# SAR-Research-Lab/lvt

Measured on AMD Instinct MI355X. Metric: stereo frames/sec (KITTI-shaped 1241x376), per-frame SE3 vs CPU ref, higher is better.
Workload: dtype u8/f64

## Files before the change

### lvt_amd/csrc/k_features.hip

```cpp
#include "lvt_dev.h"
#include "lvt_handover.h"
#include "lvt_math.h"
#include <type_traits>

namespace lvt {

__constant__ signed char c_brief[256][4] = {
#include "../../include/lvt_brief256_pattern.inc"
};
constexpr signed char BRIEF_TABLE[256][4] = {
#include "../../include/lvt_brief256_pattern.inc"
};
constexpr int brief_max_offset() {
    int m = 0;
    for (int i = 0; i < 256; i++)
        for (int k = 0; k < 4; k++) m = (BRIEF_TABLE[i][k] > m) ? BRIEF_TABLE[i][k] : (-BRIEF_TABLE[i][k] > m) ? -BRIEF_TABLE[i][k] : m;
    return m;
}

constexpr int TS_W = 64, TS_H = 16, HALO = 4;
constexpr int TILE_W = TS_W + 2 * HALO;
constexpr int TILE_H = TS_H + 2 * HALO;

typedef short s16x2 __attribute__((ext_vector_type(2)));
// ... 1786 lines not shown
constexpr int BR_WIN_DW = BR_ROWS * BR_DW, BR_LOADS = (BR_WIN_DW + 63) / 64;
template <bool BV>
__global__ __launch_bounds__(256) void k_brief(SeqArg<BV> sa, int par, seq_t publish_seq) {
    int plane, bx;
    const int planes = brief_plane_of_block(plane, bx);
    const Seq &S = sa.at(plane / gridDim.y);
    const int eye = plane % gridDim.y;
    const FrameBuf &FB = S.fb[par];
    const Feat &F = FB.feat[eye];
    const bool poison = FB.fc->poison != 0;
    const int n = poison ? 0 : *F.n;
    const int lane = lane_id();
    const int wpb = blockDim.x >> 6;
    __shared__ uint32_t s_win[4][BR_WIN_DW + 64];
    uint32_t *win = s_win[wave_id()];
    typedef uint16_t __attribute__((may_alias)) u16_alias;
    const u16_alias *win16 = reinterpret_cast<const u16_alias *>(win);
    const int W = S.prm.W, H = S.prm.H, ppd = S.plane_pitch >> 1;
    const uint32_t *box32 = reinterpret_cast<const uint32_t *>(FB.boxsum[eye]);
    int goff[BR_LOADS];
#pragma unroll
    for (int i = 0; i < BR_LOADS; i++) {
        const int e = min(lane + 64 * i, BR_WIN_DW - 1);
        goff[i] = (e / BR_DW) * ppd + (e % BR_DW);
    }
    int ta[4], tb[4];
    signed char tq[4][4];
#pragma unroll
    for (int w = 0; w < 4; w++) {
        const signed char *t = c_brief[64 * w + 8 * (lane >> 3) + 7 - (lane & 7)];
        tq[w][0] = t[0], tq[w][1] = t[1], tq[w][2] = t[2], tq[w][3] = t[3];
        ta[w] = (t[0] + BR_R) * (2 * BR_DW) + t[1] + BR_R;
        tb[w] = (t[2] + BR_R) * (2 * BR_DW) + t[3] + BR_R;
    }
    auto inside = [&](int cy, int cx) { return cx - BR_R >= 0 && cx + BR_R < W && cy - BR_R >= 0 && cy + BR_R < H; };
    int i, i_end;
    const int stride = brief_key_points_of_wave(planes, bx, wpb, n, i, i_end);
    uint32_t v[BR_LOADS];
    int cy = 0, cx = 0;
    bool fast = false;
    auto fetch = [&](int cy_, int cx_) {
        typedef const uint32_t __attribute__((address_space(1))) gu32;
        gu32 *src = (gu32 *)(box32 + (size_t)(cy_ - BR_R) * ppd + ((cx_ - BR_R) >> 1));
#pragma unroll
        for (int k = 0; k < BR_LOADS; k++) v[k] = src[goff[k]];
    };
    if (i < i_end) {
        brief_centre(F, i, cy, cx);
        fast = inside(cy, cx);
        if (fast) fetch(cy, cx);
    }
    for (; i < i_end; i += stride) {
        uint64_t word[4];
        const int inext = i + stride;
        int ncy = 0, ncx = 0;
        bool nfast = false;
        if (inext < i_end) {
            brief_centre(F, inext, ncy, ncx);
            nfast = inside(ncy, ncx);
        }
        if (fast) {
#pragma unroll
            for (int k = 0; k < BR_LOADS; k++) win[lane + 64 * k] = v[k];
            if (nfast) fetch(ncy, ncx);
            const int odd = (cx - BR_R) & 1;
#pragma unroll
            for (int w = 0; w < 4; w++) {
                const int a = win16[ta[w] + odd], b = win16[tb[w] + odd];
                word[w] = __ballot(a < b);
            }
        } else {
            if (nfast) fetch(ncy, ncx);
#pragma unroll
            for (int w = 0; w < 4; w++) {
                const int a = box_at(S, FB, eye, cy + tq[w][0], cx + tq[w][1]);
                const int b = box_at(S, FB, eye, cy + tq[w][2], cx + tq[w][3]);
                word[w] = __ballot(a < b);
            }
        }
        if (lane < 4) F.desc[(size_t)i * 4 + lane] = (lane == 0) ? word[0] : (lane == 1) ? word[1] : (lane == 2) ? word[2] : word[3];
        cy = ncy, cx = ncx, fast = nfast;
    }
    if (publish_seq) last_block_publishes(S, FB, publish_seq);
}


constexpr int BI_R = BR_R + 4, BI_ROWS = 2 * BI_R + 1;
constexpr int BI_DW = 16;
constexpr int BI_G = 13;
constexpr int BI_PATCH_DW = BI_ROWS * BI_DW, BI_LOADS = (BI_PATCH_DW + 63) / 64;
constexpr int BI_GROUPS = BI_ROWS * BI_G, BI_GLOOPS = (BI_GROUPS + 63) / 64;
template <bool BV>
__global__ __launch_bounds__(256) void k_brief_img(SeqArg<BV> sa, int par, seq_t publish_seq) {
    int plane, bx;
    const int planes = brief_plane_of_block(plane, bx);
    const Seq &S = sa.at(plane / gridDim.y);
    const int eye = plane % gridDim.y;
    const FrameBuf &FB = S.fb[par];
    const Feat &F = FB.feat[eye];
    const bool poison = FB.fc->poison != 0;
    const int n = poison ? 0 : *F.n;
    const int lane = lane_id();
    const int wpb = blockDim.x >> 6;
    __shared__ uint32_t s_patch[4][BI_PATCH_DW + 64];
    __shared__ __attribute__((aligned(8))) uint2 s_hs[4][BI_GROUPS + 64];
    uint32_t *pat = s_patch[wave_id()];
    uint2 *hs = s_hs[wave_id()];
    typedef uint16_t __attribute__((may_alias)) u16_alias;
    const u16_alias *hs16 = reinterpret_cast<const u16_alias *>(hs);
    const int W = S.prm.W, H = S.prm.H;
    const uint8_t *img = wave_uniform(FB.fc->in.img[eye]);
    const int pitch = FB.fc->in.img_pitch;
    int goff[BI_LOADS];
#pragma unroll
    for (int i = 0; i < BI_LOADS; i++) {
        const int e = min(lane + 64 * i, BI_PATCH_DW - 1);
        goff[i] = (e / BI_DW) * (pitch >> 2) + (e % BI_DW);
    }
    int ta[4], tb[4];
    signed char tq[4][4];
#pragma unroll
    for (int w = 0; w < 4; w++) {
        const signed char *t = c_brief[64 * w + 8 * (lane >> 3) + 7 - (lane & 7)];
        tq[w][0] = t[0], tq[w][1] = t[1], tq[w][2] = t[2], tq[w][3] = t[3];
        ta[w] = (t[0] + BR_R) * (4 * BI_G) + t[1] + BR_R;
        tb[w] = (t[2] + BR_R) * (4 * BI_G) + t[3] + BR_R;
    }
    auto inside = [&](int cy, int cx) { return cx - BI_R >= 0 && ((cx - BI_R) & ~3) + 64 <= pitch && cx + BI_R < W && cy - BI_R >= 0 && cy + BI_R < H; };
    int i, i_end;
    const int stride = brief_key_points_of_wave(planes, bx, wpb, n, i, i_end);
    uint32_t v[BI_LOADS];
    int cy = 0, cx = 0;
    bool fast = false;
    auto fetch = [&](int cy_, int cx_) {
        typedef const uint32_t __attribute__((address_space(1))) gu32;
        gu32 *src = (gu32 *)(reinterpret_cast<const uint32_t *>(img + (size_t)(cy_ - BI_R) * pitch) + (((cx_ - BI_R) & ~3) >> 2));
#pragma unroll
        for (int k = 0; k < BI_LOADS; k++) v[k] = src[goff[k]];
    };
    auto box_slow = [&](int iy, int ix) -> int {
        int sum = 0;
        for (int y = max(iy - 4, 0); y <= min(iy + 4, H - 1); y++)
            for (int x = max(ix - 4, 0); x <= min(ix + 4, W - 1); x++) sum += img[(size_t)y * pitch + x];
        return sum;
    };
    if (i < i_end) {
        brief_centre(F, i, cy, cx);
        fast = inside(cy, cx);
        if (fast) fetch(cy, cx);
    }
    for (; i < i_end; i += stride) {
        uint64_t word[4];
        const int inext = i + stride;
        int ncy = 0, ncx = 0;
        bool nfast = false;
        if (inext < i_end) {
            brief_centre(F, inext, ncy, ncx);
            nfast = inside(ncy, ncx);
        }
        if (fast) {
#pragma unroll
            for (int k = 0; k < BI_LOADS; k++) pat[lane + 64 * k] = v[k];
            if (nfast) fetch(ncy, ncx);
#pragma unroll
            for (int k = 0; k < BI_GLOOPS; k++) {
                const int g = min(lane + 64 * k, BI_GROUPS - 1);
// ... 36 lines not shown
```

### lvt_amd/csrc/lvt_host.hip

```cpp
#define LVT_EXPORT_FUNCTIONS
#include "../../include/lvt_amd_ext.h"

#include "k_features.hip"
#include "k_track.hip"
#include "k_hamming.hip"
#include "k_lists.hip"
#include "k_rectify.hip"
#include "k_depthreg.hip"
#include "k_equalise.hip"
#include "k_state.hip"
#include "k_poseinfo.hip"
#include "lvt_odometry.h"

#include <atomic>
#include <cmath>
#include <chrono>
#include <cstdio>
#include <cstdlib>
#include <cstring>
#include <string>
#include <functional>
#include <vector>

namespace lvt {
// ... 45 lines not shown
    const size_t head = min((size_t)(((16 - ((uintptr_t)src & 15)) & 15) / sizeof(T)), n);
    const size_t nv = (n - head) / PER, tail0 = head + nv * PER;
    const size_t t0 = (size_t)blockIdx.x * blockDim.x + threadIdx.x, stride = (size_t)gridDim.x * blockDim.x;
    for (size_t v = t0; v < nv; v += stride) {
        Vec u;
        u.q = *reinterpret_cast<const uint4 *>(src + head + v * PER);
        T *d = dst + head + v * PER;
#pragma unroll
        for (size_t k = 0; k < PER; k++) d[k] = u.e[k];
    }
    if (t0 < head) dst[t0] = src[t0];
    if (t0 < n - tail0) dst[tail0 + t0] = src[tail0 + t0];
}
static void launch_stage_copy(hipStream_t st, const uint8_t *src, float *d_dst, size_t n, int fmt) {
    if (fmt == DEPTH_U16) hipLaunchKernelGGL(k_stage_copy<uint16_t>, dim3(256), dim3(256), 0, st, reinterpret_cast<const uint16_t *>(src), reinterpret_cast<uint16_t *>(d_dst), n);
    else hipLaunchKernelGGL(k_stage_copy<float>, dim3(256), dim3(256), 0, st, reinterpret_cast<const float *>(src), d_dst, n);
}

constexpr int MAX_DEVICES = 64;
static std::atomic<int> g_live_contexts[MAX_DEVICES];
static thread_local std::string g_snap_err;

constexpr uint64_t CTX_MAGIC = 0x4C56545F43545831ull, SLOT_MAGIC = 0x4C56545F534C5431ull;

struct Rectifier {
    int w = 0, h = 0, pitch = 0;
    int device = 0;
    float *d_map1 = nullptr, *d_map2 = nullptr;
    int2 *d_fix = nullptr;
    uint8_t *d_src = nullptr, *d_dst = nullptr;
};

struct HostStage {
    uint8_t *h = nullptr, *dev = nullptr;
    size_t second = 0;
};

struct Context {
    uint64_t magic = CTX_MAGIC;
    double host_enq_us = 0, host_wait_us = 0;
    long host_enq_n = 0, host_wait_n = 0;
    int gate_timeouts_seen = 0, gate_fatal_seen = 0;
    bool want_events = false, ordering_forced = false;
    hipEvent_t ev_switch = nullptr, ev_switch_e = nullptr;
    long test_gate_timeout = 0, switched_at = -1;
    long long planes_in_place = 0, planes_staged = 0;
    int device = 0;
    int B = 1;
    int launch_seqs = 0;
    int ring_seqs[8] = {};
    int sensor = 1;
    Params prm{};
    bool mixed = false;
    std::vector<Params> prms;
    std::vector<lvt_amd_params> in_prms;
    uint32_t *d_score_tab = nullptr, *d_cells_tab = nullptr;
    int n_score_wgs = 0, n_cells_wgs = 0;
    bool any_staged = false, any_strips = false;
    int max_cells = 0;
    const Params &seq_prm(int s) const { return mixed ? prms[s] : prm; }
    hipStream_t stream = nullptr;
    hipStream_t stream_f = nullptr;
    hipStream_t stream_e = nullptr;
    bool own_stream = false;
    std::vector<void *> allocs;
    const Seq *d_seqs = nullptr;
    std::vector<Seq> h_seqs;
    std::vector<Ctl *> d_ctl;
    Ctl *h_ctl = nullptr;
    Ctl *h_ctl_dev = nullptr;
    seq_t *h_done = nullptr, *h_done_dev = nullptr;
    PoseRec *h_pose = nullptr, *h_pose_dev = nullptr;
    seq_t *h_pose_done = nullptr, *h_pose_done_dev = nullptr;
    bool binned_lists = false;
    bool early_pose = true;
    bool early_pending = false;
    FrameArgs *h_fargs = nullptr;
    bool pose_info = false;
    lvt_amd_pose_info *h_pinfo = nullptr, *h_pinfo_dev = nullptr;
    hipEvent_t ev_done[RING] = {};
    bool events_only = false;
    CellOrder cell_order;
    bool feat_pack = true;
    int brief_from_image = 0;
    int score_pieces = 1;
    bool score_pieces_auto = true;
    double gate_balance_us = 0;
    int cells_raw_cap = RAW_CAP;
    unsigned cell_token = 0;
    int cell_split = 2;
    int lists_wgs_row = LISTS_WGS_ROW, lists_wgs_map = LISTS_WGS_MAP;
    int match_blocks_batch = 32;
    bool force_row_fallback = false;
    hipEvent_t ev_feat[NPAR] = {};
    hipEvent_t ev_depth = nullptr;
    bool depth_wait = false;
    std::function<void()> before_gather;
    uint8_t *d_img[NPAR][2] = {};
    HostStage stage[NPAR];
    float *d_depth[NPAR] = {};
    uint8_t *d_img_ring[RING][2] = {};
    float *d_depth_ring[RING] = {};
    HostStage stage_ring[RING];
    long long async_frames = 0;
    struct PendingFrame {
        bool valid = false, pulled = false;
        FrameArgs f{};
        const uint8_t *src[2] = {nullptr, nullptr};
        uint8_t *dst[2] = {nullptr, nullptr};
        int row_bytes = 0, pitch = 0;
    } pend;
    NextPull next_pull{};
    bool fuse_pull = true;
    long long fused_pulls = 0;
    int feature_cus = 0;
    float *d_ext[NPAR][2] = {};
    std::vector<Rectifier *> rect;
    std::vector<uint8_t *> d_rect;
    int n_rect = 0;
    bool has_rect(int s) const { return n_rect > 0 && rect[2 * (size_t)s] != nullptr; }
    std::vector<int> pixfmt;
    std::vector<uint8_t *> d_gray;
    int n_colour = 0;
    bool ring_converted[RING] = {};
    int fmt_of(int s) const { return n_colour > 0 ? pixfmt[(size_t)s] : PIX_GRAY8; }
    int bpp_of(int s) const { return pix_bpp(fmt_of(s)); }
    uint8_t *d_col[NPAR][2] = {};
    uint8_t *d_col_ring[RING][2] = {};
    int colour_pitch() const { return (prm.W * bpp_of(0) + 63) / 64 * 64; }
    std::vector<lvt_amd_depth_camera> depth_cam;
    std::vector<float *> d_reg;
    int n_depth_cam = 0;
    bool ring_registered[RING] = {};
    bool has_depth_cam(int s) const { return n_depth_cam > 0 && depth_cam[(size_t)s].width > 0; }
    std::vector<lvt_amd_equalisation> equal;
    std::vector<uint8_t *> d_eq;
    std::vector<uint8_t *> d_eq_lut;
    int n_equal = 0;
    bool ring_equalised[RING] = {};
    bool has_equal(int s) const { return n_equal > 0 && equal[(size_t)s].tiles_x > 0; }
    size_t depth_px() const { return has_depth_cam(0) ? (size_t)depth_cam[0].width * depth_cam[0].height : (size_t)prm.W * prm.H; }
    int depth_cols() const { return has_depth_cam(0) ? depth_cam[0].width : prm.W; }
    size_t depth_cap = 0, depth_ring_cap = 0;
    int pitch = 0;
    int *d_snap_status = nullptr;
    long enq = 0, done = 0;
    long delivered = 0;
    bool sync_call = false;
    int last_slot = 0, last_par = 0;
    std::string err;
    bool prof = false;
    static constexpr int PROF_SLOTS = 26;
    hipEvent_t ev[PROF_SLOTS][2] = {};
    bool ev_used[PROF_SLOTS] = {};
    double prof_ms[PROF_SLOTS] = {};
    long prof_calls[PROF_SLOTS] = {};

    void set_error(const std::string &s) { err = s; }
    long long ovf_done = -1, ovf_read_done = -1;
    bool capacity_report() const { return err.compare(0, 17, "capacity overflow") == 0; }

    template <typename T>
    T *dalloc_uncached(size_t n) {
        void *p = nullptr;
        size_t bytes = ((n * sizeof(T) + 255) / 256) * 256;
        if (bytes == 0) bytes = 256;
// ... 289 lines not shown
    c->device = device;
    DeviceGuard guard(c);
    try {
        c->count_in(device);
        c->B = B;
        c->sensor = sensor;
        c->prm = prm;
        c->mixed = mixed;
        if (mixed) c->prms = prms;
        c->in_prms.assign(in, in + prms.size());
        for (const Params &q : prms) {
            c->any_staged = c->any_staged || q.staged_th > 0;
            c->any_strips = c->any_strips || q.big_cell_strips != 0;
            c->max_cells = std::max(c->max_cells, q.n_cells);
        }
        HIPCHK(c, hipStreamCreateWithFlags(&c->stream, hipStreamNonBlocking));
        {
            int ncu = 0;
            if (B >= 2 && B <= 28) {
                int total = 0;
                if (hipDeviceGetAttribute(&total, hipDeviceAttributeMultiprocessorCount, device) == hipSuccess && total >= 64) ncu = total / 8 * 7;
            }
            if (const char *e = std::getenv("LVT_AMD_FEATURE_CUS")) ncu = (B >= 2) ? std::atoi(e) : 0;
            if (ncu > 0 && ncu < 1024) {
                uint32_t mask[32] = {};
                for (int i = 0; i < ncu; i++) mask[i >> 5] |= 1u << (i & 31);
                HIPCHK(c, hipExtStreamCreateWithCUMask(&c->stream_f, 32, mask));
                c->feature_cus = ncu;
            } else
                HIPCHK(c, hipStreamCreateWithFlags(&c->stream_f, hipStreamNonBlocking));
        }
        HIPCHK(c, hipStreamCreateWithFlags(&c->stream_e, hipStreamNonBlocking));
        c->own_stream = true;
        for (auto &e : c->ev_done) HIPCHK(c, hipEventCreateWithFlags(&e, hipEventDisableTiming));
        for (auto &e : c->ev_feat) HIPCHK(c, hipEventCreateWithFlags(&e, hipEventDisableTiming));
        HIPCHK(c, hipEventCreateWithFlags(&c->ev_depth, hipEventDisableTiming));
        HIPCHK(c, hipEventCreateWithFlags(&c->ev_switch, hipEventDisableTiming));
        HIPCHK(c, hipEventCreateWithFlags(&c->ev_switch_e, hipEventDisableTiming));
        if (const char *e = std::getenv("LVT_AMD_TEST_GATE_TIMEOUT")) c->test_gate_timeout = std::atol(e);
        {
            const char *o = std::getenv("LVT_AMD_ORDERING");
            if (o && std::strcmp(o, "events") == 0) c->events_only = true;
            else if (o && std::strcmp(o, "polling") == 0) c->events_only = false, c->ordering_forced = true;
            else c->events_only = B == 1 && c->live_on_device() > 1;
        }
        c->pitch = ((prm.W + 63) / 64) * 64;
        HIPCHK(c, hipHostMalloc((void **)&c->h_ctl, sizeof(Ctl) * B * RING, hipHostMallocCoherent));
        HIPCHK(c, hipHostGetDevicePointer((void **)&c->h_ctl_dev, c->h_ctl, 0));
        HIPCHK(c, hipHostMalloc((void **)&c->h_done, sizeof(seq_t) * B * RING, hipHostMallocCoherent));
        HIPCHK(c, hipHostGetDevicePointer((void **)&c->h_done_dev, c->h_done, 0));
        std::memset(c->h_done, 0, sizeof(seq_t) * B * RING);
        HIPCHK(c, hipHostMalloc((void **)&c->h_pose, sizeof(PoseRec) * B * RING, hipHostMallocCoherent));
        HIPCHK(c, hipHostGetDevicePointer((void **)&c->h_pose_dev, c->h_pose, 0));
        HIPCHK(c, hipHostMalloc((void **)&c->h_pose_done, sizeof(seq_t) * B * RING, hipHostMallocCoherent));
        HIPCHK(c, hipHostGetDevicePointer((void **)&c->h_pose_done_dev, c->h_pose_done, 0));
        std::memset(c->h_pose_done, 0, sizeof(seq_t) * B * RING);
        if (const char *e = std::getenv("LVT_AMD_SYNC_TAIL")) c->early_pose = std::strcmp(e, "wait") != 0;
        c->binned_lists = B > 1;
        if (const char *e = std::getenv("LVT_AMD_BINNED_LISTS")) c->binned_lists = std::atoi(e) != 0;
        if (const char *e = std::getenv("LVT_AMD_TEST_ROW_FALLBACK")) c->force_row_fallback = std::atoi(e) != 0;
        {
            int idx[CELLS_MAX], area[CELLS_MAX];
            for (int cc = 0; cc < prm.n_cells; cc++) {
                const int cx = cc % prm.cells_x, cy = cc / prm.cells_x;
                idx[cc] = cc;
                area[cc] = std::min(prm.cell_size, prm.W - cx * prm.cell_size) * std::min(prm.cell_size, prm.H - cy * prm.cell_size);
            }
            std::stable_sort(idx, idx + prm.n_cells, [&](int a, int b) { return area[a] > area[b]; });
            for (int cc = 0; cc < CELLS_MAX; cc++) c->cell_order.v[cc] = (uint8_t)(cc < prm.n_cells ? idx[cc] : 0);
        }
        if (std::getenv("LVT_AMD_NO_FEAT_PACK")) c->feat_pack = false;
        if (const char *e = std::getenv("LVT_AMD_BRIEF_FROM_IMAGE")) c->brief_from_image = std::atoi(e) ? 1 : 0;
        if (const char *e = std::getenv("LVT_AMD_SCORE_PIECES")) c->score_pieces = std::max(1, std::min(8, std::atoi(e))), c->score_pieces_auto = false;
        {
            int n_cu = 256;
            (void)hipDeviceGetAttribute(&n_cu, hipDeviceAttributeMultiprocessorCount, c->device);
            if (!mixed && !prm.big_cell_strips && prm.n_cells * 2 * B > n_cu) c->cells_raw_cap = RAW_CAP_SMALL;
            if (mixed && !c->any_strips && (int)cells_tab.size() > n_cu) c->cells_raw_cap = RAW_CAP_SMALL;
        }
        if (mixed) c->score_pieces = 1, c->score_pieces_auto = false;
        if (const char *e = std::getenv("LVT_AMD_CELL_SPLIT")) c->cell_split = std::max(0, std::min(SPLIT_MAX, std::atoi(e)));
        if (const char *e = std::getenv("LVT_AMD_CELLS_RAW_CAP")) c->cells_raw_cap = std::max(RAW_CAP_SMALL, std::min(RAW_CAP, std::atoi(e) & ~1));
        if (const char *e = std::getenv("LVT_AMD_FUSED_PULL")) c->fuse_pull = std::atoi(e) != 0;
        c->lists_wgs_row = c->lists_wgs_map = (B <= 16) ? 4 : 2;
        if (const char *e = std::getenv("LVT_AMD_LISTS_WGS")) {
            int r = 0, m = 0;
            const int got = std::sscanf(e, "%d,%d", &r, &m);
            if (got >= 1) c->lists_wgs_row = std::max(1, std::min(64, r));
            if (got >= 2) c->lists_wgs_map = std::max(1, std::min(64, m));
        }
        if (const char *e = std::getenv("LVT_AMD_MATCH_BLOCKS_BATCH")) c->match_blocks_batch = std::max(1, std::min(256, std::atoi(e)));
        HIPCHK(c, hipHostMalloc((void **)&c->h_fargs, sizeof(FrameArgs) * B * RING, hipHostMallocDefault));
        std::memset(c->h_fargs, 0, sizeof(FrameArgs) * B * RING);
        c->h_seqs.resize(B);
        c->d_ctl.resize(B);
        for (int s = 0; s < B; s++) {
            const Params &q = prms[mixed ? s : 0];
            const int pitch = ((q.W + 63) / 64) * 64;
            const size_t plane = (size_t)pitch * q.H;
            Seq &S = c->h_seqs[s];
            std::memset(&S, 0, sizeof(S));
            S.prm = q;
            S.ctl = c->d_ctl[s] = c->dalloc<Ctl>(1);
            S.plane_pitch = pitch;
            {
                size_t off = 0;
                for (int cc = 0; cc < q.n_cells; cc++) {
                    const int cx = cc % q.cells_x, cy = cc / q.cells_x;
                    const int cw = std::min(q.cell_size, q.W - cx * q.cell_size), ch = std::min(q.cell_size, q.H - cy * q.cell_size);
                    S.cell_scratch_off[cc] = off;
                    off += (size_t)cw * ch * 6;
                }
            }
            for (int e = 0; e < 2; e++) S.cell_scratch[e] = c->dalloc<uint32_t>((size_t)q.W * q.H * 6 + 64);
            for (int e = 0; e < 2; e++) {
                S.strip_kp[e] = q.big_cell_strips ? c->dalloc<uint32_t>((size_t)q.n_cells * STRIPS * RAW_CAP) : c->dalloc_uncached<uint32_t>((size_t)q.n_cells * SPLIT_MAX * SPLIT_KP_CAP);
                S.strip_n[e] = c->dalloc_uncached<int>((size_t)CELLS_MAX * STRIPS);
                S.cell_big[e] = c->dalloc<int>(CELLS_MAX);
            }
            S.lists_fb = c->dalloc<int>(2);
            for (int par = 0; par < NPAR; par++) {
                FrameBuf &FB = S.fb[par];
                FB.fc = c->dalloc<FeatCtl>(1);
                for (int e = 0; e < 2; e++) {
                    FB.score[e] = c->dalloc<uint8_t>(plane + 64);
                    FB.boxsum[e] = c->dalloc<uint16_t>(plane + 64);
                    {
                        const size_t tiles_x = (size_t)(q.W + TS_W - 1) / TS_W;
                        FB.seg_keys[e] = c->dalloc<uint32_t>((size_t)q.H * tiles_x * TS_W);
                        FB.seg_cnt[e] = c->dalloc<uint16_t>((size_t)q.H * tiles_x);
                    }
                    FB.cell_kp[e] = c->dalloc<float>((size_t)CELLS_MAX * CELL_OUT_CAP * 3);
                    FB.cell_n[e] = c->dalloc<int>(CELLS_MAX);
                    alloc_feat(c, FB.feat[e]);
                    if (s == 0) {
                        c->d_ext[par][e] = c->dalloc<float>((size_t)EXT_MAX * 2);
                        c->d_img[par][e] = c->dalloc<uint8_t>(plane + 64);
                    }
                    FB.ext_xy_own[e] = c->d_ext[par][e];
                }
                if (s == 0 && sensor == 2) c->d_depth[par] = c->dalloc<float>((size_t)q.W * q.H + 4), c->depth_cap = (size_t)q.W * q.H;
            }
            for (int k = 0; k < 2; k++) {
                alloc_points(c, S.map[k], MAP_MAX);
                alloc_points(c, S.staged[k], STAGED_MAX);
            }
            S.map_cur = c->dalloc<int>(1), S.map_n = c->dalloc<int>(1);
            S.staged_cur = c->dalloc<int>(1), S.staged_n = c->dalloc<int>(1);
            S.proj = c->dalloc<float>((size_t)MAP_MAX * 2);
            S.vis = c->dalloc<int8_t>(MAP_MAX);
            S.match = c->dalloc<int>(MAP_MAX);
            S.cand = c->dalloc<uint32_t>((size_t)MAP_MAX * KC);
            S.ncand = c->dalloc<int>(MAP_MAX);
            S.qidx = c->dalloc<uint32_t>(MAP_MAX);
            S.sproj = c->dalloc<float>((size_t)STAGED_MAX * 2);
            S.svis = c->dalloc<int8_t>(STAGED_MAX);
            S.smatch = c->dalloc<int>(STAGED_MAX);
            S.scand = c->dalloc<uint32_t>((size_t)STAGED_MAX * KC);
            S.sncand = c->dalloc<int>(STAGED_MAX);
            S.sdel = c->dalloc<uint8_t>(STAGED_MAX);
            S.pnp_X = c->dalloc<double>((size_t)NF_MAX * 3);
            S.pnp_obs = c->dalloc<float>((size_t)NF_MAX * 2);
            S.pnp_feat = c->dalloc<int>(NF_MAX);
            S.pnp_err = c->dalloc<double>((size_t)NF_MAX * 2 + 2);
            S.pnp_level = c->dalloc<int8_t>(NF_MAX);
            S.rcand = c->dalloc<uint32_t>((size_t)NPAR * NF_MAX * KC);
            S.rncand = c->dalloc<int>(NPAR * NF_MAX);
            S.pair_l = c->dalloc<int>(NF_MAX), S.pair_r = c->dalloc<int>(NF_MAX);
            S.tri_X = c->dalloc<double>((size_t)NF_MAX * 3);
            S.tri_ok = c->dalloc<int8_t>(NF_MAX);
        }
        {
            Seq *d = c->dalloc<Seq>(B);
            HIPCHK(c, hipMemcpy(d, c->h_seqs.data(), sizeof(Seq) * B, hipMemcpyHostToDevice));
            c->d_seqs = d;
        }
        if (mixed) {
            c->n_score_wgs = (int)score_tab.size(), c->n_cells_wgs = (int)cells_tab.size();
            c->d_score_tab = c->dalloc<uint32_t>(score_tab.size());
            c->d_cells_tab = c->dalloc<uint32_t>(cells_tab.size());
            HIPCHK(c, hipMemcpy(c->d_score_tab, score_tab.data(), sizeof(uint32_t) * score_tab.size(), hipMemcpyHostToDevice));
            HIPCHK(c, hipMemcpy(c->d_cells_tab, cells_tab.data(), sizeof(uint32_t) * cells_tab.size(), hipMemcpyHostToDevice));
            HIPCHK(c, hipFuncSetAttribute(reinterpret_cast<const void *>(&k_cells_mixed), hipFuncAttributeMaxDynamicSharedMemorySize, CELLS_LDS_BYTES));
        }
        HIPCHK(c, hipFuncSetAttribute(reinterpret_cast<const void *>(&k_cells<true>), hipFuncAttributeMaxDynamicSharedMemorySize, CELLS_LDS_BYTES));
        HIPCHK(c, hipFuncSetAttribute(reinterpret_cast<const void *>(&k_cells<false>), hipFuncAttributeMaxDynamicSharedMemorySize, CELLS_LDS_BYTES));
        HIPCHK(c, hipFuncSetAttribute(reinterpret_cast<const void *>(&k_hamming_batched_lists<MODE_MAP, true>), hipFuncAttributeMaxDynamicSharedMemorySize, LS_LDS_BYTES));
        HIPCHK(c, hipFuncSetAttribute(reinterpret_cast<const void *>(&k_hamming_batched_lists<MODE_MAP, false>), hipFuncAttributeMaxDynamicSharedMemorySize, LS_LDS_BYTES));
        HIPCHK(c, hipFuncSetAttribute(reinterpret_cast<const void *>(&k_hamming_batched_lists<MODE_ROW, true>), hipFuncAttributeMaxDynamicSharedMemorySize, LS_LDS_BYTES));
        HIPCHK(c, hipFuncSetAttribute(reinterpret_cast<const void *>(&k_hamming_batched_lists<MODE_ROW, false>), hipFuncAttributeMaxDynamicSharedMemorySize, LS_LDS_BYTES));
        HIPCHK(c, hipFuncSetAttribute(reinterpret_cast<const void *>(&k_cells_strip), hipFuncAttributeMaxDynamicSharedMemorySize, CELLS_LDS_BYTES));
        HIPCHK(c, hipFuncSetAttribute(reinterpret_cast<const void *>(&k_gather<true>), hipFuncAttributeMaxDynamicSharedMemorySize, CELLS_LDS_BYTES));
        HIPCHK(c, hipFuncSetAttribute(reinterpret_cast<const void *>(&k_gather<false>), hipFuncAttributeMaxDynamicSharedMemorySize, CELLS_LDS_BYTES));
        HIPCHK(c, hipFuncSetAttribute(reinterpret_cast<const void *>(&k_cells_big), hipFuncAttributeMaxDynamicSharedMemorySize, CELLS_LDS_BYTES));
        HIPCHK(c, hipFuncSetAttribute(reinterpret_cast<const void *>(&k_cells_radii), hipFuncAttributeMaxDynamicSharedMemorySize, CELLS_LDS_BYTES));
        HIPCHK(c, hipFuncSetAttribute(reinterpret_cast<const void *>(&k_cells_select), hipFuncAttributeMaxDynamicSharedMemorySize, CELLS_LDS_BYTES));
        HIPCHK(c, hipFuncSetAttribute(reinterpret_cast<const void *>(&k_pnp<true>), hipFuncAttributeMaxDynamicSharedMemorySize, PNP_DYN_BYTES));
        HIPCHK(c, hipFuncSetAttribute(reinterpret_cast<const void *>(&k_pnp<false>), hipFuncAttributeMaxDynamicSharedMemorySize, PNP_DYN_BYTES));
        reset_state(c);
    } catch (...) {
        delete c;
        return nullptr;
    }
    return c;
}
static Context *create_context(const lvt_amd_params &in, int sensor, int B, int device = -1) { return create_context(&in, false, sensor, B, device); }

static const char *kProfNames[Context::PROF_SLOTS] = {
    "k_feat_begin", "k_gate [early stream: waits for the previous k_pnp]", "k_score", "k_cells(pass0)", "k_rectify_frames", "k_gather(+ the rare retry pass)", "k_brief", "k_gate_late [waits for the early stream]",
    "k_match_map(wait for the early stream + begin + new points)", "k_early_map [early stream]", "k_early_mid [early stream]", "k_hamming_batched_lists(map) [early stream]", "k_track_mid(resolve+pass2+bookkeep+cull)", "k_pnp(+project staged)", "k_gray_frames",
    "k_pose_info", "k_candidates(staged)", "k_depth_clear", "k_candidates(row) [early stream]", "k_hamming_batched_lists(row)", "k_triangulate(staged update+row resolve+triangulate+finalize)", "k_depth_register",
    "k_state_pack", "k_state_unpack", "k_clahe_lut", "k_clahe_apply"};

#define LAUNCH(slot, st, kern, grid, block, lds, ...)                              \
    do {                                                                           \
        if (c->prof) (void)hipEventRecord(c->ev[slot][0], st);                     \
        hipLaunchKernelGGL(kern, grid, block, lds, st, __VA_ARGS__);               \
        if (c->prof) {                                                             \
            (void)hipEventRecord(c->ev[slot][1], st);                              \
            c->ev_used[slot] = true;                                               \
        }                                                                          \
    } while (0)

#define LAUNCH_S(slot, st, kern, grid, block, lds, ...)                                                      \
    do {                                                                                                     \
        if (B == 1) LAUNCH(slot, st, kern<true>, grid, block, lds, SeqArg<true>{c->h_seqs[0]}, __VA_ARGS__); \
        else LAUNCH(slot, st, kern<false>, grid, block, lds, SeqArg<false>{S}, __VA_ARGS__);                  \
    } while (0)
#define LAUNCH_SM(slot, st, kern, MODE_, grid, block, lds, ...)                                                        \
    do {                                                                                                               \
        if (B == 1) LAUNCH(slot, st, (kern<MODE_, true>), grid, block, lds, SeqArg<true>{c->h_seqs[0]}, __VA_ARGS__);   \
        else LAUNCH(slot, st, (kern<MODE_, false>), grid, block, lds, SeqArg<false>{S}, __VA_ARGS__);                   \
    } while (0)

static void collect_oldest(Context *c);

static FrameArgs stereo_args(const void *left, const void *right, int pitch_bytes) {
    FrameArgs f{};
    f.img[0] = static_cast<const uint8_t *>(left);
    f.img[1] = static_cast<const uint8_t *>(right);
    f.img_pitch = pitch_bytes;
    return f;
}
static FrameArgs with_depth(FrameArgs f, const void *depth, int depth_pitch_bytes, int fmt, float scale) {
    f.depth = static_cast<const float *>(depth);
    f.depth_pitch = depth_pitch_bytes / ((fmt == DEPTH_U16) ? 2 : 4);
    f.depth_format = fmt;
    f.depth_scale = (fmt == DEPTH_U16) ? scale : 0.f;
    return f;
}
static FrameArgs rgbd_args(const void *gray, int gray_pitch, const void *depth, int depth_pitch_bytes, int fmt, float scale) {
    return with_depth(stereo_args(gray, gray, gray_pitch), depth, depth_pitch_bytes, fmt, scale);
}
static FrameArgs absent_args() {
    FrameArgs f{};
    f.absent = 1;
    return f;
}
static FrameArgs with_corners(FrameArgs f, int n_left, int n_right, const float *xy_left = nullptr, const float *xy_right = nullptr) {
    f.ext_corners = 1;
    f.n_ext[0] = n_left, f.n_ext[1] = n_right;
    f.ext_xy[0] = xy_left, f.ext_xy[1] = xy_right;
    return f;
}
static FrameArgs &frame_args(Context *c, int slot, int s = 0) { return c->h_fargs[(size_t)slot * c->B + s]; }
static int next_slot(const Context *c) { return (int)(c->enq % RING); }

struct HostTimer {
    double *acc;
    std::chrono::steady_clock::time_point t0;
    explicit HostTimer(double *a) : acc(a), t0(std::chrono::steady_clock::now()) {}
    ~HostTimer() { *acc += std::chrono::duration<double, std::micro>(std::chrono::steady_clock::now() - t0).count(); }
};
static seq_t buffer_last_user(const Context *c) { return (seq_t)(c->enq + 1 - NPAR); }
struct DepthRegStep {
    DepthRegTable tab;
// ... 19 lines not shown
    const Seq *S = c->d_seqs;
    const int slot = (int)(c->enq % RING), par = (int)(c->enq % NPAR);
    if (c->want_events && !c->events_only) {
        if (c->enq > 0 && c->delivered < c->enq) {
            const int pslot = (int)((c->enq - 1) % RING);
            hipLaunchKernelGGL(k_deliver, dim3(1, 1, Bz), dim3(64), 0, c->stream, S, c->h_ctl_dev + (size_t)pslot * B, c->h_done_dev + (size_t)pslot * B, (seq_t)c->enq);
            c->delivered = c->enq;
        }
        (void)hipEventRecord(c->ev_switch_e, c->stream_e);
        (void)hipStreamWaitEvent(c->stream, c->ev_switch_e, 0);
        (void)hipStreamWaitEvent(c->stream_f, c->ev_switch_e, 0);
        (void)hipEventRecord(c->ev_switch, c->stream);
        (void)hipStreamWaitEvent(c->stream_f, c->ev_switch, 0);
        c->events_only = true;
        c->want_events = false;
        c->switched_at = (long)c->enq;
    }
    const FrameArgs *fa = &frame_args(c, slot);
    const int ext = (B == 1) ? fa[0].ext_corners : 0;
    hipStream_t sf = c->stream_f, st = c->stream;
    for (int i = 0; i < Context::PROF_SLOTS; i++) c->ev_used[i] = false;
    c->ring_converted[slot] = c->ring_registered[slot] = c->ring_equalised[slot] = false;
    if (c->n_colour) convert_colour_frames(c, slot, par, Bz);
    if (c->n_rect) rectify_raw_frames(c, slot, par, Bz);
    if (c->n_equal) equalise_frames(c, slot, par, Bz);
    DepthRegPlan dreg;
    if (c->n_depth_cam) begin_depth_registration(c, slot, par, Bz, dreg);
    const bool evo = c->events_only;
    const bool feat_pack = B > 1 && Bz <= FEAT_PACK && c->feat_pack;
    if (c->enq >= NPAR) {
        if (!evo) {
            if (!feat_pack) hipLaunchKernelGGL(k_gate_buf, dim3(1, 1, Bz), dim3(64), 0, sf, S, buffer_last_user(c), par);
        } else if (c->switched_at < 0 || (long)c->enq - NPAR >= c->switched_at) {
            (void)hipStreamWaitEvent(sf, c->ev_done[(int)((c->enq - NPAR) % RING)], 0);
        }
    }
    if (B == 1) {
        LAUNCH(2, sf, k_score<true>, dim3((p.W + TS_W - 1) / TS_W, (p.H + TS_H - 1) / TS_H, 2), dim3(256), 0, S, c->h_fargs[slot], par, 0, c->brief_from_image ? 0 : 1);
    } else {
        if (feat_pack) {
            FrameArgsPack pk;
            std::memset(&pk, 0, sizeof(pk));
            for (int s = 0; s < Bz; s++) pk.a[s] = fa[s];
            LAUNCH(0, sf, k_feat_begin_pack, dim3(Bz), dim3(64), 0, S, pk, par, (c->enq >= NPAR && !evo) ? buffer_last_user(c) : (seq_t)0);
        } else
            LAUNCH(0, sf, k_feat_begin, dim3(Bz), dim3(64), 0, S, fa, par);
        if (c->mixed) {
            LAUNCH(2, sf, k_score_mixed, dim3(c->n_score_wgs), dim3(256), 0, S, c->d_score_tab, par, c->brief_from_image ? 0 : 1);
        } else {
            const int P = std::max(1, std::min(c->score_pieces, Bz));
            for (int q = 0; q < P; q++) {
                const int z0 = 2 * (int)((long)Bz * q / P), z1 = 2 * (int)((long)Bz * (q + 1) / P);
                if (q == 0) LAUNCH(2, sf, k_score<false>, dim3((p.W + TS_W - 1) / TS_W, (p.H + TS_H - 1) / TS_H, z1 - z0), dim3(256), 0, S, FrameArgs{}, par, z0, c->brief_from_image ? 0 : 1);
                else hipLaunchKernelGGL(k_score<false>, dim3((p.W + TS_W - 1) / TS_W, (p.H + TS_H - 1) / TS_H, z1 - z0), dim3(256), 0, sf, S, FrameArgs{}, par, z0, c->brief_from_image ? 0 : 1);
            }
        }
    }
    if (!ext) {
        {
            const int pull_wgs = (B == 1 && c->next_pull.src[0]) ? std::min(64, (int)(((size_t)c->next_pull.W * c->next_pull.H / 16 + 1023) / 1024)) : 0;
            const int ns = (B == 1 && !p.big_cell_strips) ? c->cell_split : 0;
            const int gx = (ns >= 2) ? ((((p.n_cells + 7) & ~7) * ns + pull_wgs + 7) & ~7) : p.n_cells + pull_wgs;
            if (c->mixed) LAUNCH(3, sf, k_cells_mixed, dim3(c->n_cells_wgs), dim3(1024), cells_lds_bytes(c->cells_raw_cap), S, c->d_cells_tab, par, c->cells_raw_cap);
            else LAUNCH_S(3, sf, k_cells, (B == 1 ? dim3(gx, 2, 1) : dim3(p.n_cells * 2 * Bz, 1, 1)), dim3(1024), cells_lds_bytes(c->cells_raw_cap), par, c->cell_order, 2 * Bz, c->cells_raw_cap, c->next_pull, ns, (++c->cell_token ? c->cell_token : ++c->cell_token));
            if (c->any_strips) {
                const int nc = c->max_cells;
                hipLaunchKernelGGL(k_cells_strip, dim3(nc * STRIPS, 2, Bz), dim3(1024), CELLS_LDS_BYTES, sf, S, par);
                hipLaunchKernelGGL(k_cells_big, dim3(nc, 2, Bz), dim3(1024), CELLS_LDS_BYTES, sf, S, par);
                hipLaunchKernelGGL(k_cells_radii, dim3(nc * RADII_WGS, 2, Bz), dim3(1024), CELLS_LDS_BYTES, sf, S, par);
                hipLaunchKernelGGL(k_cells_select, dim3(nc, 2, Bz), dim3(1024), CELLS_LDS_BYTES, sf, S, par);
                if (c->prof) (void)hipEventRecord(c->ev[3][1], sf);
            }
        }
    }
    if (c->before_gather) {
        c->before_gather();
        c->before_gather = nullptr;
    }
    if (c->depth_wait) {
        (void)hipStreamWaitEvent(sf, c->ev_depth, 0);
        c->depth_wait = false;
    }
    scatter_depth_planes(c, dreg);
    LAUNCH_S(5, sf, k_gather, dim3(1, 2, Bz), dim3(1024), CELLS_LDS_BYTES, par);
    const bool brief_publishes = !evo && B == 1;
    if (c->brief_from_image) LAUNCH_S(6, sf, k_brief_img, dim3(64, 2, Bz), dim3(256), 0, par, brief_publishes ? (seq_t)(c->enq + 1) : (seq_t)0);
    else LAUNCH_S(6, sf, k_brief, dim3(64, 2, Bz), dim3(256), 0, par, brief_publishes ? (seq_t)(c->enq + 1) : (seq_t)0);
    if (!evo && !brief_publishes) hipLaunchKernelGGL(k_feat_done, dim3(Bz), dim3(64), 0, sf, S, par, (seq_t)(c->enq + 1));
    const int bl = c->binned_lists ? 1 : 0;
    if (evo && bl && c->sensor == 1) LAUNCH_SM(19, sf, k_hamming_batched_lists, MODE_ROW, dim3(c->lists_wgs_row, 1, Bz), dim3(LS_THREADS), LS_LDS_BYTES, par, (seq_t)0);
    if (evo) LAUNCH_SM(18, sf, k_candidates, MODE_ROW, dim3(256, 1, Bz), dim3(256), 0, 0, par, (seq_t)0, bl);
    if (evo) hipLaunchKernelGGL(k_feat_done, dim3(Bz), dim3(64), 0, sf, S, par, (seq_t)(c->enq + 1));
    if (evo) (void)hipEventRecord(c->ev_feat[par], sf);
    const seq_t seq = (seq_t)(c->enq + 1);
    if (!evo) {
        hipStream_t se = c->stream_e;
        LAUNCH_S(1, se, k_gate, dim3(1, 1, Bz), dim3(64), 0, par, (seq_t)c->enq, seq, (c->test_gate_timeout && (long)seq == c->test_gate_timeout) ? 1 : 0);
        if (bl) LAUNCH_SM(11, se, k_hamming_batched_lists, MODE_MAP, dim3(c->lists_wgs_map, 1, Bz), dim3(LS_THREADS), LS_LDS_BYTES, par, seq);
        LAUNCH_S(9, se, k_early_map, dim3((bl && B > 1) ? 32 : 256, 1, Bz), dim3(256), 0, par, seq, bl);
        LAUNCH_S(10, se, k_early_mid, dim3(1, 1, Bz), dim3(RES_THREADS), 0, par, seq);
        if (c->sensor == 1) {
            if (bl) LAUNCH_SM(19, se, k_hamming_batched_lists, MODE_ROW, dim3(c->lists_wgs_row, 1, Bz), dim3(LS_THREADS), LS_LDS_BYTES, par, seq);
            LAUNCH_SM(18, se, k_candidates, MODE_ROW, dim3(B == 1 ? ROW_BLOCKS : ROW_BLOCKS_BATCH, 1, Bz), dim3(256), 0, 0, par, seq, bl);
            hipLaunchKernelGGL(k_row_done, dim3(Bz), dim3(64), 0, se, S, par, seq);
        }
    }
    {
        Ctl *prec = nullptr;
        seq_t *pdone = nullptr;
        if (!evo && c->delivered < c->enq) {
            const int pslot = (int)((c->enq - 1) % RING);
            prec = c->h_ctl_dev + (size_t)pslot * B, pdone = c->h_done_dev + (size_t)pslot * B;
            c->delivered = c->enq;
        }
        if (evo) {
            (void)hipStreamWaitEvent(st, c->ev_feat[par], 0);
            LAUNCH_S(8, st, k_match_map, dim3(256, 1, Bz), dim3(256), 0, par, seq, 0, (Ctl *)nullptr, (seq_t *)nullptr);
        } else if (B == 1 && c->live_on_device() <= MAX_FOLDED_GATES) {
            LAUNCH_S(8, st, k_match_map, dim3(MATCH_BLOCKS_GATED, 1, 1), dim3(256), 0, par, seq, 1, prec, pdone);
        } else {
            LAUNCH_S(7, st, k_gate_late, dim3(1, 1, Bz), dim3(64), 0, par, seq, prec, pdone);
            LAUNCH_S(8, st, k_match_map, dim3(B > 1 ? c->match_blocks_batch : 256, 1, Bz), dim3(256), 0, par, seq, 0, (Ctl *)nullptr, (seq_t *)nullptr);
        }
    }
    LAUNCH_S(12, st, k_track_mid, dim3(1, 1, Bz), dim3(RES_THREADS), 0, par, seq);
    {
        const bool ep = c->sync_call && c->early_pose && !c->prof && B == 1;
        LAUNCH_S(13, st, k_pnp, dim3(1, 1, Bz), dim3(PNP_THREADS), PNP_DYN_BYTES, par, seq, ep ? c->h_pose_dev + (size_t)slot * B : (PoseRec *)nullptr,
                 ep ? c->h_pose_done_dev + (size_t)slot * B : (seq_t *)nullptr);
    }
    if (c->pose_info) LAUNCH_S(15, st, k_pose_info, dim3(1, 1, Bz), dim3(PI_THREADS), 0, c->h_pinfo_dev + (size_t)slot * B);
    if (c->any_staged)
        LAUNCH_SM(16, st, k_candidates, MODE_STAGED, dim3(64, 1, Bz), dim3(256), 0, 0, par, (seq_t)0, 0);
    LAUNCH_S(20, st, k_triangulate, dim3(1, 1, Bz), dim3(1024), 0, par, seq, c->h_ctl_dev + (size_t)slot * B,
           c->h_done_dev + (size_t)slot * B, evo ? 0 : (c->force_row_fallback ? 2 : 1), (evo || c->sync_call) ? 1 : 0);
    if (evo || c->sync_call) c->delivered = c->enq + 1;
    if (evo) (void)hipEventRecord(c->ev_done[slot], st);
    c->enq++;
}

enum class SpinStop { FLAG_A, FLAG_B, STREAM_ERROR, STREAM_IDLE };
static SpinStop spin_on_flags(Context *c, seq_t want, volatile seq_t *a, volatile seq_t *b, unsigned &spins, hipError_t *q) {
    for (;;) {
        if (__atomic_load_n(a, __ATOMIC_ACQUIRE) == want) return SpinStop::FLAG_A;
        if (b && __atomic_load_n(b, __ATOMIC_ACQUIRE) == want) return SpinStop::FLAG_B;
        __builtin_ia32_pause();
        if ((++spins & 0xFFFFF) == 0) {
            *q = hipStreamQuery(c->stream);
            if (*q != hipErrorNotReady) return *q == hipSuccess ? SpinStop::STREAM_IDLE : SpinStop::STREAM_ERROR;
        }
    }
}
static void collect_oldest(Context *c) {
    HostTimer ht(&c->host_wait_us);
    c->host_wait_n++;
    if (c->done >= c->enq) return;
    const int slot = (int)(c->done % RING);
    const int Bz = (c->ring_seqs[slot] > 0 && c->ring_seqs[slot] <= c->B) ? c->ring_seqs[slot] : c->B;
    if (c->delivered < c->done + 1) {
        hipLaunchKernelGGL(k_deliver, dim3(1, 1, Bz), dim3(64), 0, c->stream, c->d_seqs, c->h_ctl_dev + (size_t)slot * c->B,
                           c->h_done_dev + (size_t)slot * c->B, (seq_t)(c->done + 1));
        c->delivered = c->done + 1;
    }
    {
        const seq_t want = (seq_t)(c->done + 1);
        unsigned spins = 0;
        for (int s = 0; s < Bz; s++) {
            volatile seq_t *f = c->h_done + (size_t)slot * c->B + s;
            hipError_t q = hipSuccess;
// ... 2055 lines not shown
```

Baseline: 9139.

## Fuse keypoint gather into wide 1024-thread BRIEF kernel for single-sequence stereo

Measured after the change: 8390. 0.918x the previous value.

```diff
diff --git a/lvt_amd/csrc/k_features.hip b/lvt_amd/csrc/k_features.hip
--- a/lvt_amd/csrc/k_features.hip
+++ b/lvt_amd/csrc/k_features.hip
@@ -1892,6 +1892,174 @@
         cy = ncy, cx = ncx, fast = nfast;
     }
     if (publish_seq) last_block_publishes(S, FB, publish_seq);
+}
+
+constexpr int BW_WAVES = 16, BW_GRID_X = 64;
+constexpr int BW_STRIDE = (BW_GRID_X >> 3) * BW_WAVES;
+constexpr int BW_KP = ((NF_MAX + 7) / 8 + BW_STRIDE - 1) / BW_STRIDE;
+constexpr int BW_WIN_BYTES = BW_WAVES * (BR_WIN_DW + 64) * 4;
+constexpr int BW_OFF_DW = 80;
+constexpr int BW_LDS_BYTES = BW_WIN_BYTES + NF_MAX * 4 + BW_OFF_DW * 4 + 64 * 4;
+constexpr int BW_GATHER_U = 2;
+static_assert(CELLS_MAX + 1 <= BW_OFF_DW && CELLS_MAX <= 64 && BW_WIN_BYTES % 16 == 0 && BW_WAVES * BW_KP <= NF_MAX && BW_KP <= 64, "k_brief_wide's LDS carve");
+
+__device__ __forceinline__ uint32_t brief_centre_word(float by, float bx) { return (uint32_t)(int)((double)by + 0.5) << 16 | (uint32_t)(int)((double)bx + 0.5); }
+
+__device__ __forceinline__ int brief_gather(const Seq &S, const FrameBuf &FB, int eye, bool writer, uint32_t *cen, int *cell_off, int *scan) {
+    constexpr int U = BW_GATHER_U, TRIP = U * 64 * BW_WAVES;
+    FeatCtl &ctl = *FB.fc;
+    const Feat &F = FB.feat[eye];
+    const int tid = threadIdx.x;
+    const int nc = S.prm.n_cells;
+    if (tid < 64) {
+        const int incl = wave_incl_scan(tid < nc ? FB.cell_n[eye][tid] : 0);
+        cell_off[tid + 1] = incl;
+        if (tid == 0) cell_off[0] = 0;
+    }
+    __syncthreads();
+    const int total_in = cell_off[nc];
+    const int W = S.prm.W, H = S.prm.H;
+    int n_out = 0;
+    for (int base = 0; base < total_in; base += TRIP) {
+        float x[U], y[U], r[U];
+        int c = 0;
+#pragma unroll
+        for (int u = 0; u < U; u++) {
+            const int g = base + tid * U + u;
+            x[u] = y[u] = r[u] = 0.f;
+            if (g < total_in) {
+                while (g >= cell_off[c + 1]) c++;
+                const float *kp = FB.cell_kp[eye] + ((size_t)c * CELL_OUT_CAP + (g - cell_off[c])) * 3;
+                x[u] = kp[0], y[u] = kp[1], r[u] = kp[2];
+            }
+        }
+        unsigned keep = 0;
+#pragma unroll
+        for (int u = 0; u < U; u++)
+            if (base + tid * U + u < total_in && brief_border_keep(x[u], y[u], H, W)) keep |= 1u << u;
+        int total;
+        int off = n_out + block_excl_scan(__popc(keep), scan, &total);
+#pragma unroll
+        for (int u = 0; u < U; u++) {
+            if (!(keep >> u & 1)) continue;
+            if (off < NF_MAX) {
+                cen[off] = brief_centre_word(y[u], x[u]);
+                if (writer) {
+                    F.x[off] = x[u];
+                    F.y[off] = y[u];
+                    F.resp[off] = r[u];
+                    F.bx[off] = x[u];
+                    F.by[off] = y[u];
+                    F.depth[off] = 0.f;
+                    F.flag[off] = 0;
+                    F.hcy[off] = (int16_t)floorf(y[u] / (float)HASH_CELL);
+                    F.hcx[off] = (int16_t)floorf(x[u] / (float)HASH_CELL);
+                }
+            }
+            off++;
+        }
+        n_out += total;
+    }
+    if (writer && tid == 0) {
+        if (n_out > NF_MAX) atomicOr(&ctl.overflow, OVF_FEATURES);
+        *F.n = min(n_out, NF_MAX);
+    }
+    __syncthreads();
+    return min(n_out, NF_MAX);
+}
+
+template <bool GATHER>
+__global__ __launch_bounds__(64 * BW_WAVES) void k_brief_wide(SeqArg<true> sa, int par, seq_t publish_seq) {
+    int plane, bx;
+    const int planes = brief_plane_of_block(plane, bx);
+    const Seq &S = sa.get();
+    const int eye = plane % gridDim.y;
+    const FrameBuf &FB = S.fb[par];
+    const Feat &F = FB.feat[eye];
+    const bool poison = FB.fc->poison != 0;
+    const int lane = lane_id();
+    extern __shared__ __attribute__((aligned(16))) uint8_t smem[];
+    uint32_t *win = reinterpret_cast<uint32_t *>(smem) + wave_id() * (BR_WIN_DW + 64);
+    uint32_t *s_cen = reinterpret_cast<uint32_t *>(smem + BW_WIN_BYTES);
+    int *s_off = reinterpret_cast<int *>(s_cen + NF_MAX);
+    typedef uint16_t __attribute__((may_alias)) u16_alias;
+    const u16_alias *win16 = reinterpret_cast<const u16_alias *>(win);
+    const int W = S.prm.W, H = S.prm.H, ppd = S.plane_pitch >> 1;
+    const uint32_t *box32 = reinterpret_cast<const uint32_t *>(FB.boxsum[eye]);
+    int n = 0;
+    if (!poison) n = GATHER ? brief_gather(S, FB, eye, bx == 0, s_cen, s_off, s_off + BW_OFF_DW) : *F.n;
+    int i, i_end;
+    const int stride = brief_key_points_of_wave(planes, bx, BW_WAVES, n, i, i_end);
+    const uint32_t *cen = s_cen + i;
+    int cstep = stride;
+    if (!GATHER) {
+        uint32_t *mine = s_cen + wave_id() * BW_KP;
+        const int ik = i + lane * stride;
+        if (lane < BW_KP && ik < i_end) mine[lane] = brief_centre_word(F.by[ik], F.bx[ik]);
+        cen = mine, cstep = 1;
+    }
+    int goff[BR_LOADS];
+#pragma unroll
+    for (int q = 0; q < BR_LOADS; q++) {
+        const int e = min(lane + 64 * q, BR_WIN_DW - 1);
+        goff[q] = (e / BR_DW) * ppd + (e % BR_DW);
+    }
+    int ta[4], tb[4];
+#pragma unroll
+    for (int w = 0; w < 4; w++) {
+        const signed char *t = c_brief[64 * w + 8 * (lane >> 3) + 7 - (lane & 7)];
+        ta[w] = (t[0] + BR_R) * (2 * BR_DW) + t[1] + BR_R;
+        tb[w] = (t[2] + BR_R) * (2 * BR_DW) + t[3] + BR_R;
+    }
+    auto inside = [&](uint32_t c) { const int cy = (int)(c >> 16), cx = (int)(c & 0xffff); return cx - BR_R >= 0 && cx + BR_R < W && cy - BR_R >= 0 && cy + BR_R < H; };
+    const int count = i < i_end ? (i_end - i + stride - 1) / stride : 0;
+    auto centre = [&](int k) { return wave_uniform(cen[min(k, BW_KP - 1) * cstep]); };
+    uint32_t v[BR_LOADS];
+    auto fetch = [&](uint32_t c) {
+        typedef const uint32_t __attribute__((address_space(1))) gu32;
+        const int cy_ = (int)(c >> 16), cx_ = (int)(c & 0xffff);
+        gu32 *src = (gu32 *)(box32 + (size_t)(cy_ - BR_R) * ppd + ((cx_ - BR_R) >> 1));
+#pragma unroll
+        for (int q = 0; q < BR_LOADS; q++) v[q] = src[goff[q]];
+    };
+    if (count > 0 && inside(centre(0))) fetch(centre(0));
+    for (int k = 0; k < count; k++) {
+        const uint32_t cur = centre(k);
+        uint64_t word[4] = {0, 0, 0, 0};
+        const bool fast = inside(cur);
+        if (fast) {
+#pragma unroll
+            for (int q = 0; q < BR_LOADS; q++) win[lane + 64 * q] = v[q];
+        }
+        if (k + 1 < count) {
+            const uint32_t next = centre(k + 1);
+            if (inside(next)) fetch(next);
+        }
+        if (fast) {
+            const int odd = ((int)(cur & 0xffff) - BR_R) & 1;
+#pragma unroll
+            for (int w = 0; w < 4; w++) {
+                const int a = win16[ta[w] + odd], b = win16[tb[w] + odd];
+                word[w] = __ballot(a < b);
+            }
+        }
+        if (lane < 4) F.desc[(size_t)(i + k * stride) * 4 + lane] = (lane == 0) ? word[0] : (lane == 1) ? word[1] : (lane == 2) ? word[2] : word[3];
+    }
+    if (publish_seq) last_block_publishes(S, FB, publish_seq);
+}
+
+__global__ __launch_bounds__(1024) void k_retry(SeqArg<true> sa, int par) {
+    const Seq &S = sa.get();
+    const int eye = blockIdx.y;
+    const FrameBuf &FB = S.fb[par];
+    FeatCtl &ctl = *FB.fc;
+    if (ctl.n_detected[eye] >= CORNERS_LOW_TH || ctl.poison) return;
+    extern __shared__ __attribute__((aligned(16))) uint8_t smem[];
+    const CellLds L = carve_cell_lds(smem);
+    for (int cell = 0; cell < S.prm.n_cells; cell++) {
+        cells_work(S, FB, eye, cell, 1, L);
+        __syncthreads();
+    }
 }
 
 
diff --git a/lvt_amd/csrc/lvt_host.hip b/lvt_amd/csrc/lvt_host.hip
--- a/lvt_amd/csrc/lvt_host.hip
+++ b/lvt_amd/csrc/lvt_host.hip
@@ -151,6 +151,8 @@
     bool events_only = false;
     CellOrder cell_order;
     bool feat_pack = true;
+    bool brief_wide = true;
+    bool brief_gather = true;
     int brief_from_image = 0;
     int score_pieces = 1;
     bool score_pieces_auto = true;
@@ -606,6 +608,8 @@
         if (const char *e = std::getenv("LVT_AMD_CELL_SPLIT")) c->cell_split = std::max(0, std::min(SPLIT_MAX, std::atoi(e)));
         if (const char *e = std::getenv("LVT_AMD_CELLS_RAW_CAP")) c->cells_raw_cap = std::max(RAW_CAP_SMALL, std::min(RAW_CAP, std::atoi(e) & ~1));
         if (const char *e = std::getenv("LVT_AMD_FUSED_PULL")) c->fuse_pull = std::atoi(e) != 0;
+        if (const char *e = std::getenv("LVT_AMD_BRIEF_WIDE")) c->brief_wide = std::atoi(e) != 0;
+        if (const char *e = std::getenv("LVT_AMD_BRIEF_GATHER")) c->brief_gather = std::atoi(e) != 0;
         c->lists_wgs_row = c->lists_wgs_map = (B <= 16) ? 4 : 2;
         if (const char *e = std::getenv("LVT_AMD_LISTS_WGS")) {
             int r = 0, m = 0;
@@ -716,6 +720,9 @@
         HIPCHK(c, hipFuncSetAttribute(reinterpret_cast<const void *>(&k_cells_strip), hipFuncAttributeMaxDynamicSharedMemorySize, CELLS_LDS_BYTES));
         HIPCHK(c, hipFuncSetAttribute(reinterpret_cast<const void *>(&k_gather<true>), hipFuncAttributeMaxDynamicSharedMemorySize, CELLS_LDS_BYTES));
         HIPCHK(c, hipFuncSetAttribute(reinterpret_cast<const void *>(&k_gather<false>), hipFuncAttributeMaxDynamicSharedMemorySize, CELLS_LDS_BYTES));
+        HIPCHK(c, hipFuncSetAttribute(reinterpret_cast<const void *>(&k_retry), hipFuncAttributeMaxDynamicSharedMemorySize, CELLS_LDS_BYTES));
+        HIPCHK(c, hipFuncSetAttribute(reinterpret_cast<const void *>(&k_brief_wide<true>), hipFuncAttributeMaxDynamicSharedMemorySize, BW_LDS_BYTES));
+        HIPCHK(c, hipFuncSetAttribute(reinterpret_cast<const void *>(&k_brief_wide<false>), hipFuncAttributeMaxDynamicSharedMemorySize, BW_LDS_BYTES));
         HIPCHK(c, hipFuncSetAttribute(reinterpret_cast<const void *>(&k_cells_big), hipFuncAttributeMaxDynamicSharedMemorySize, CELLS_LDS_BYTES));
         HIPCHK(c, hipFuncSetAttribute(reinterpret_cast<const void *>(&k_cells_radii), hipFuncAttributeMaxDynamicSharedMemorySize, CELLS_LDS_BYTES));
         HIPCHK(c, hipFuncSetAttribute(reinterpret_cast<const void *>(&k_cells_select), hipFuncAttributeMaxDynamicSharedMemorySize, CELLS_LDS_BYTES));
@@ -901,9 +908,14 @@
         c->depth_wait = false;
     }
     scatter_depth_planes(c, dreg);
-    LAUNCH_S(5, sf, k_gather, dim3(1, 2, Bz), dim3(1024), CELLS_LDS_BYTES, par);
     const bool brief_publishes = !evo && B == 1;
-    if (c->brief_from_image) LAUNCH_S(6, sf, k_brief_img, dim3(64, 2, Bz), dim3(256), 0, par, brief_publishes ? (seq_t)(c->enq + 1) : (seq_t)0);
+    const bool wide = brief_publishes && c->brief_wide && c->sensor == 1 && !ext && !c->brief_from_image && c->live_on_device() <= MAX_FOLDED_GATES;
+    const bool fused_gather = wide && c->brief_gather;
+    if (fused_gather) LAUNCH(5, sf, k_retry, dim3(1, 2, 1), dim3(1024), CELLS_LDS_BYTES, SeqArg<true>{c->h_seqs[0]}, par);
+    else LAUNCH_S(5, sf, k_gather, dim3(1, 2, Bz), dim3(1024), CELLS_LDS_BYTES, par);
+    if (fused_gather) LAUNCH(6, sf, k_brief_wide<true>, dim3(BW_GRID_X, 2, 1), dim3(64 * BW_WAVES), BW_LDS_BYTES, SeqArg<true>{c->h_seqs[0]}, par, (seq_t)(c->enq + 1));
+    else if (wide) LAUNCH(6, sf, k_brief_wide<false>, dim3(BW_GRID_X, 2, 1), dim3(64 * BW_WAVES), BW_LDS_BYTES, SeqArg<true>{c->h_seqs[0]}, par, (seq_t)(c->enq + 1));
+    else if (c->brief_from_image) LAUNCH_S(6, sf, k_brief_img, dim3(64, 2, Bz), dim3(256), 0, par, brief_publishes ? (seq_t)(c->enq + 1) : (seq_t)0);
     else LAUNCH_S(6, sf, k_brief, dim3(64, 2, Bz), dim3(256), 0, par, brief_publishes ? (seq_t)(c->enq + 1) : (seq_t)0);
     if (!evo && !brief_publishes) hipLaunchKernelGGL(k_feat_done, dim3(Bz), dim3(64), 0, sf, S, par, (seq_t)(c->enq + 1));
     const int bl = c->binned_lists ? 1 : 0;
```
